# vvvm23/distributed-pytorch-cookbook

Measured on AMD Instinct MI355X. Metric: tokens/sec (node) GPT-2 training per recipe (DDP/FSDP/PP) at 1/2/4/8 MI355X, higher is better.
Workload: dtype bf16; 1 GPU; model=gpt2-small, global_batch=64, seq_len=1024, parallelism=dp1, recipe=main-ddp.py, reduce_dtype=fp32, pp_comm_dtype=fp32, step_graph=True

## Files before the change

distributed_pytorch_cookbook_amd/models/fused.py:

```python
from __future__ import annotations

import os
from dataclasses import dataclass
from typing import Optional

import torch

from ..ops.attention import attention_bwd, attention_fwd
from ..ops.elementwise import bias_act_bwd
from ..ops.dropout import dropout_residual
from ..ops.embedding import embedding_bwd, embedding_fwd
from ..ops.gemm import (ACT_GELU, ACT_MUL, ACT_NONE, ACT_RELU, act_code, linear_dgrad, linear_fwd, linear_wgrad,
                        register_side_stream)
from ..ops.loss import cross_entropy_fused, cross_entropy_rows
from ..ops.norm import layernorm_bwd, layernorm_fwd

LN_EPS = 1e-5
_DH_F32 = os.environ.get("DPC_DH_F32", "0") == "1"


def _dh_dtype(cdt):
    return torch.float32 if _DH_F32 else cdt


_HEAD_DGRAD_F32 = os.environ.get("DPC_HEAD_DGRAD_F32", "auto")


def _head_dgrad_dtype(T, D, cdt):
    if _HEAD_DGRAD_F32 in ("0", "1"):
        return torch.float32 if _HEAD_DGRAD_F32 == "1" else _dh_dtype(cdt)
    tiles = ((T + 255) // 256) * ((D + 255) // 256)
    return torch.float32 if tiles < 128 else _dh_dtype(cdt)


_HEAD_CHUNK = int(os.environ.get("DPC_HEAD_CHUNK", "0"))


def vocab_ld(vocab: int) -> int:
    return (vocab + 63) // 64 * 64


@dataclass
class LMOutput:
    loss: torch.Tensor
    n_valid: torch.Tensor
    n_correct: Optional[torch.Tensor] = None


def _qkv_weight(store, attn):
    wq, wk, wv = (store.weight(m.weight) for m in (attn.to_q, attn.to_k, attn.to_v))
    n = wq.shape[0]
    if (wk.data_ptr() == wq.data_ptr() + wq.numel() * wq.element_size()
            and wv.data_ptr() == wk.data_ptr() + wk.numel() * wk.element_size()):
        return wq.as_strided((3 * n, wq.shape[1]), (wq.shape[1], 1))
    return torch.cat([wq, wk, wv], 0)


def _head_weight_padded(store, head, rows: int):
    w = store.weight(head.weight)
    V, D = w.shape
    if rows == V or getattr(head.weight, "_dpc_pad_rows", 0) == 0 or w.stride() != (D, 1):
        return w
    end = w.storage_offset() + rows * D
    if end * w.element_size() > w.untyped_storage().nbytes():
        return w
    return w.as_strided((rows, D), (D, 1))
# ... 141 lines not shown

_FUSE_TAIL = os.environ.get("DPC_FUSE_FFN_TAIL", "1") == "1"
_FUSE_FFN_LN = os.environ.get("DPC_FUSE_FFN_LN", "1") == "1"


def _tail_ok(x, cdt):
    return _FUSE_TAIL and (cdt == torch.bfloat16 or not x.is_cuda)


class _LayerFn(torch.autograd.Function):

    @staticmethod
    def forward(ctx, x, mask, layer, store, N, S, act, training, drops=(None, None), recompute=False,
                prev_tail=None, tail=None):
        u = layer._unit_id
        store.pre_forward(u)
        pre = None
        if prev_tail is not None and prev_tail.pending is not None:
            pre, prev_tail.pending = prev_tail.pending, None
        fuse = tail if (tail is not None and tail.fuse_next) else None
        x3, saved = _layer_forward(x, mask, layer, store, N, S, act, training and not recompute, drops,
                                   pre=pre, fuse_out=fuse)
        store.post_forward(u, training)
        if training:
            ctx.save_for_backward(x, mask, *(saved or ()))
            ctx.layer, ctx.store, ctx.dims, ctx.act = layer, store, (N, S), act
            ctx.drops, ctx.recompute = drops, recompute
            ctx.fused_out = fuse is not None
            ctx.prev_tail, ctx.tail = prev_tail, tail
            if tail is not None and saved is not None and _tail_ok(x, store.compute_dtype):
                tail.z2, tail.act, tail.drop = saved[-1], act, drops[1]
                bias = layer.fc.down_proj.bias
                tail.bias_grad = lambda: store.grad(bias)
        return x3

    @staticmethod
    def backward(ctx, dx3):
        x, mask, *saved = ctx.saved_tensors
        layer, store, act = ctx.layer, ctx.store, ctx.act
        N, S = ctx.dims
        H, hd = layer.attn.heads, layer.attn.head_dim
        store.pre_backward(layer._unit_id)
        if ctx.recompute:
            _, saved = _layer_forward(x, mask, layer, store, N, S, act, True, ctx.drops,
                                      fuse_out=_FfnTail() if ctx.fused_out else None)
        dx = _layer_backward(dx3, x, mask, saved, layer, store, N, S, H, hd, act, ctx.drops,
                             ctx.prev_tail, ctx.tail)
        u = layer._unit_id
        _w(lambda: store.post_backward(u))
        return dx, None, None, None, None, None, None, None, None, None, None, None


_WGRAD_STREAM = os.environ.get("DPC_WGRAD_STREAM", "0") == "1"
_side_streams: dict = {}


class _SideWork:
    def __init__(self, device: torch.device):
        self.on = _WGRAD_STREAM and device.type == "cuda"
        self.stream = None
        if self.on:
            key = torch.cuda.current_stream(device).cuda_stream
            if key not in _side_streams:
                _side_streams[key] = torch.cuda.Stream(device=device)
                register_side_stream(_side_streams[key])
            self.stream = _side_streams[key]

    def run(self, fn, *tensors):
        if _W_DEFER is not None:
            _W_DEFER.append(fn)
            return
        if not self.on:
            fn()
            return
        self.stream.wait_stream(torch.cuda.current_stream(self.stream.device))
        with torch.cuda.stream(self.stream):
            fn()
        for t in tensors:
            t.record_stream(self.stream)

    def join(self):
        if self.on:
            torch.cuda.current_stream(self.stream.device).wait_stream(self.stream)


def _layer_backward(dx3, x, mask, saved, layer, store, N, S, H, hd, act, drops, prev_tail=None, tail=None):
    (h1, mu1, rs1, qkv, o, lse, x2, h2, mu2, rs2, zup, uact, z2) = saved
    attn, fc = layer.attn, layer.fc
    w, g = store.weight, store.grad
    cdt = store.compute_dtype
    drop_attn, drop_ffn = drops
    dx = dx3.contiguous()
    side = _SideWork(dx.device)
    if tail is not None and tail.dz2 is not None:
        dz2 = tail.dz2
        tail.dz2 = None
    else:
        dz2 = bias_act_bwd(dx, z2, act, g(fc.down_proj.bias), out_dtype=cdt, drop=drop_ffn)
    side.run(lambda: linear_wgrad(dz2, uact, out=g(fc.down_proj.weight)), dz2, uact)
    dz1 = linear_dgrad(dz2, w(fc.down_proj.weight), act_bwd=ACT_MUL if act == ACT_GELU else act, aux_in=zup,
                       out_dtype=cdt, colsum=g(fc.up_proj.bias))
    side.run(lambda: linear_wgrad(dz1, h2, out=g(fc.up_proj.weight)), dz1, h2)
    dh2 = linear_dgrad(dz1, w(fc.up_proj.weight), out_dtype=_dh_dtype(cdt))
    dyo = torch.empty(dx.shape, device=dx.device, dtype=cdt)
    layernorm_bwd(dh2, x2, mu2, rs2, w(layer.norm2.weight), dx, g(layer.norm2.weight),
                  g(layer.norm2.bias), gout=dyo, gsum=g(attn.to_out.bias), drop=drop_attn)
    side.run(lambda: linear_wgrad(dyo, o, out=g(attn.to_out.weight)), dyo, o)
    do = linear_dgrad(dyo, w(attn.to_out.weight), out_dtype=cdt)
    dqkv = attention_bwd(do, qkv, o, lse, N, S, H, hd, mask, causal=True)
    gqkv, split = _qkv_grad(store, attn)

    def qkv_wgrad():
        linear_wgrad(dqkv, h1, out=gqkv)
        if split is not None:
            n = split[0].shape[0]
            for i, gi in enumerate(split):
                gi.add_(gqkv[i * n:(i + 1) * n])

    side.run(qkv_wgrad, dqkv, h1, gqkv)
    dh1 = linear_dgrad(dqkv, _qkv_weight(store, attn), out_dtype=_dh_dtype(cdt))
    kw = {}
    if prev_tail is not None:
        prev_tail.consume(kw, x.shape[0], x.shape[1], x.device, cdt)
    layernorm_bwd(dh1, x, mu1, rs1, w(layer.norm1.weight), dx, g(layer.norm1.weight),
                  g(layer.norm1.bias), **kw)
    side.join()
    return dx


def _ln_in(x, pending, gamma, beta, cdt):
    if pending is None:
        return layernorm_fwd(x, gamma, beta, LN_EPS, cdt)
    x2p, z2p, dropp, actp = pending
    return layernorm_fwd(x2p, gamma, beta, LN_EPS, cdt, add=(z2p, None, dropp, actp), x_out=x)


_unit_ln = {}


def materialize_pending(x, tail) -> None:
    if tail is None or tail.pending is None:
        return
    pending, tail.pending = tail.pending, None
    D = x.shape[1]
    key = (x.device, D)
    if key not in _unit_ln:
        _unit_ln[key] = (torch.ones(D, device=x.device), torch.zeros(D, device=x.device))
    g, b = _unit_ln[key]
    with torch.no_grad():
        _ln_in(x, pending, g, b, pending[1].dtype)


class _HeadFn(torch.autograd.Function):

    @staticmethod
    def forward(ctx, x, targets, norm, head, store, unit, training, want_correct, prev_tail=None):
        store.pre_forward(unit)
        w = store.weight
        cdt = store.compute_dtype
        V = w(head.weight).shape[0]
        T = x.shape[0]
        pending = None
        if prev_tail is not None and prev_tail.pending is not None:
            pending, prev_tail.pending = prev_tail.pending, None
        hf, mu, rs = _ln_in(x, pending, w(norm.weight), w(norm.bias), cdt)
        ld = vocab_ld(V) if x.is_cuda else V
        buf = torch.empty(T, ld, device=x.device, dtype=cdt)
        wpad = _head_weight_padded(store, head, ld)
        chunk = _HEAD_CHUNK if (x.is_cuda and cdt == torch.bfloat16) else 0
        if chunk and T > chunk:
            tg = targets.reshape(-1)
            n_valid = (tg != -100).sum().float()
            inv = 1.0 / n_valid.clamp_min(1.0)
            row_loss = torch.empty(T, device=x.device, dtype=torch.float32)
            row_corr = torch.empty(T, device=x.device, dtype=torch.float32) if want_correct else None
            for c0 in range(0, T, chunk):
                c1 = min(T, c0 + chunk)
                linear_fwd(hf[c0:c1], wpad, out=buf[c0:c1])
# ... 124 lines not shown
```

distributed_pytorch_cookbook_amd/ops/_lib.py:

```python
from __future__ import annotations

import ctypes
import os
import threading
from ctypes import c_float, c_int, c_longlong, c_uint, c_void_p

import torch

from . import build as _build

P = c_void_p
LL = c_longlong


class GemmArgs(ctypes.Structure):
    _fields_ = [
        ("A", P), ("B", P), ("C", P), ("bias", P), ("residual", P), ("aux_in", P),
        ("aux_out", P), ("alpha_ptr", P), ("colsum", P),
        ("lda", LL), ("ldb", LL), ("ldc", LL), ("ldr", LL), ("ld_aux_in", LL), ("ld_aux_out", LL),
        ("M", c_int), ("N", c_int), ("K", c_int),
        ("alpha", c_float),
        ("act", c_int), ("act_bwd", c_int), ("out_f32", c_int), ("accumulate", c_int),
        ("a_kmaj", c_int), ("b_kmaj", c_int),
        ("a_r", c_int), ("a_c", c_int), ("b_r", c_int), ("b_c", c_int),
# ... 187 lines not shown
    "dpc_decode_attn": DecodeAttnArgs,
    "dpc_gemv": GemvArgs,
    "dpc_sample": SampleArgs,
    "dpc_embedding_bwd_sorted": EmbBwdArgs,
    "dpc_gemm": GemmArgs,
    "dpc_gemm_f32": GemmArgs,
    "dpc_attn_fwd": AttnArgs,
    "dpc_attn_bwd": AttnArgs,
    "dpc_attn_fwd_f32": AttnArgs,
    "dpc_attn_bwd_f32": AttnArgs,
    "dpc_layernorm_fwd": LNArgs,
    "dpc_layernorm_bwd": LNArgs,
    "dpc_embedding_fwd": EmbArgs,
    "dpc_embedding_bwd": EmbArgs,
    "dpc_cross_entropy": CEArgs,
    "dpc_adamw": AdamArgs,
    "dpc_amp_check": AmpCheckArgs,
    "dpc_amp_update": AmpUpdateArgs,
    "dpc_grad_sumsq": GradSumsqArgs,
    "dpc_clip_coef": ClipCoefArgs,
    "dpc_cast_f32_bf16": CastArgs,
    "dpc_bias_act_bwd": BiasActArgs,
    "dpc_dropout_residual": DropResArgs,
}

_lock = threading.Lock()
_lib = None
_error = None


def lib() -> ctypes.CDLL:
    global _lib, _error
    if _lib is not None:
        return _lib
    if _error is not None:
        raise RuntimeError(f"kernel library unavailable: {_error}")
    with _lock:
        if _lib is None:
            if _build.needs_build():
                try:
                    _build.build()
                except Exception as exc:
                    _error = exc
                    raise
            handle = ctypes.CDLL(str(_build.LIB_PATH), mode=ctypes.RTLD_GLOBAL)
            for name, st in _FUNCS.items():
                fn = getattr(handle, name)
                fn.argtypes = [ctypes.POINTER(st), c_void_p]
                fn.restype = c_int
            handle.dpc_gemm_set_impl.argtypes = [c_int]
            handle.dpc_gemm_set_impl.restype = None
            handle.dpc_gemm_explain.argtypes = [ctypes.POINTER(GemmArgs), ctypes.c_char_p, c_int]
            handle.dpc_gemm_explain.restype = c_int
            handle.dpc_gemm_last_kernel.argtypes = []
            handle.dpc_gemm_last_kernel.restype = c_int
            handle.dpc_gemm_set_xcd_split.argtypes = [c_int]
            handle.dpc_gemm_set_xcd_split.restype = None
            handle.dpc_gemm_set_splits.argtypes = [c_int]
            handle.dpc_gemm_set_splits.restype = None
            handle.dpc_set_cu_reserve.argtypes = [c_int]
            handle.dpc_set_cu_reserve.restype = None
            handle.dpc_get_cu_reserve.argtypes = []
            handle.dpc_get_cu_reserve.restype = c_int
            handle.dpc_occupy.argtypes = [c_int, ctypes.c_longlong, c_void_p, c_void_p]
            handle.dpc_occupy.restype = c_int
            handle.dpc_embedding_bwd_ws.argtypes = [c_int, c_int]
            handle.dpc_embedding_bwd_ws.restype = ctypes.c_ulonglong
            handle.dpc_grad_sumsq_max_blocks.argtypes = []
            handle.dpc_grad_sumsq_max_blocks.restype = c_int
            handle.dpc_grad_sumsq_trip.argtypes = []
            handle.dpc_grad_sumsq_trip.restype = ctypes.c_longlong
            if (handle.dpc_grad_sumsq_max_blocks(), handle.dpc_grad_sumsq_trip()) != (SUMSQ_MAX_BLOCKS, SUMSQ_TRIP):
                raise RuntimeError("kernel library: dpc_grad_sumsq geometry differs from ops/_lib.py")
            handle.dpc_ipc_alloc.argtypes = [ctypes.c_longlong, c_int, ctypes.POINTER(c_void_p)]
            handle.dpc_ipc_free.argtypes = [c_void_p]
            handle.dpc_ipc_handle.argtypes = [c_void_p, c_void_p]
            handle.dpc_ipc_open.argtypes = [c_void_p, ctypes.POINTER(c_void_p)]
            handle.dpc_ipc_close.argtypes = [c_void_p]
            handle.dpc_ipc_coll.argtypes = [ctypes.POINTER(IpcCollArgs), c_void_p]
            handle.dpc_ipc_p2p.argtypes = [ctypes.POINTER(IpcP2PArgs), c_void_p]
            for f in ("dpc_ipc_alloc", "dpc_ipc_free", "dpc_ipc_handle", "dpc_ipc_open", "dpc_ipc_close",
                      "dpc_ipc_coll", "dpc_ipc_p2p", "dpc_ipc_handle_size", "dpc_ipc_max_world", "dpc_ipc_groups"):
                getattr(handle, f).restype = c_int
            _lib = handle
    return _lib


forced_gemm_impl = -1


def set_gemm_impl(impl: int) -> None:
    global forced_gemm_impl
    forced_gemm_impl = int(impl)
    lib().dpc_gemm_set_impl(int(impl))


def gemm_last_kernel() -> int:
    return int(lib().dpc_gemm_last_kernel())


def gemm_explain(args: GemmArgs) -> str:
    buf = ctypes.create_string_buffer(1024)
    lib().dpc_gemm_explain(ctypes.byref(args), buf, len(buf))
    return buf.value.decode()


def set_gemm_splits(n: int) -> None:
    lib().dpc_gemm_set_splits(int(n))


def set_gemm_xcd_split(on: bool) -> None:
    lib().dpc_gemm_set_xcd_split(int(bool(on)))


def set_cu_reserve(r: int) -> None:
    lib().dpc_set_cu_reserve(int(r))


def get_cu_reserve() -> int:
    return int(lib().dpc_get_cu_reserve())


def occupy(nwg: int, ns: int, sink: torch.Tensor, stream=None) -> None:
    s = (stream or torch.cuda.current_stream()).cuda_stream
    rc = lib().dpc_occupy(int(nwg), int(ns), sink.data_ptr(), s)
    if rc != 0:
        raise RuntimeError(f"dpc_occupy failed: hipError {rc}")


def is_loaded() -> bool:
    return _lib is not None


def stream_ptr(device: torch.device | None = None) -> int:
    return torch.cuda.current_stream(device).cuda_stream


SERIALIZE = os.environ.get("DPC_SERIALIZE", "0") == "1"


def enable_serialize() -> None:
    global SERIALIZE
    SERIALIZE = True
    os.environ["DPC_SERIALIZE"] = "1"
    for k, v in (("AMD_SERIALIZE_KERNEL", "3"), ("AMD_SERIALIZE_COPY", "3"), ("HIP_LAUNCH_BLOCKING", "1")):
        os.environ.setdefault(k, v)


def call(name: str, args: ctypes.Structure, device: torch.device | None = None) -> None:
    rc = getattr(lib(), name)(ctypes.byref(args), stream_ptr(device))
    if rc != 0:
        raise RuntimeError(f"{name} launch failed: hipError {rc}")
    if SERIALIZE and not torch.cuda.is_current_stream_capturing():
        try:
            torch.cuda.current_stream(device).synchronize()
        except RuntimeError as exc:
            raise RuntimeError(f"{name} failed on the device: {exc}") from exc


# ... 3 lines not shown
```

distributed_pytorch_cookbook_amd/ops/build.py:

```python
from __future__ import annotations

import argparse
import os
import shutil
import subprocess
import sys
from concurrent.futures import ThreadPoolExecutor
from pathlib import Path

HERE = Path(__file__).resolve().parent
CSRC = HERE / "csrc"
BUILD_DIR = HERE / "_build"
LIB_PATH = HERE / "libdpc_kernels.so"
ARCH = os.environ.get("DPC_OFFLOAD_ARCH", "gfx950")

SOURCES = ["gemm.hip", "gemm_f32.hip", "attention.hip", "attention_f32.hip", "layernorm.hip", "misc.hip",
           "decode.hip", "sample.hip", "embed_bwd.hip", "ipc_coll.hip"] + sorted(p.name for p in CSRC.glob("gemm7_part*.hip"))
HEADERS = ["common.h", "gemm.h", "gemm_plan.h", "gemm7_kern.h", "gemm9_kern.h", "gemm7_extern.inc"]

CFLAGS = [
    f"--offload-arch={ARCH}",
    "-O3",
    "-std=c++17",
    "-fPIC",
    "-mcode-object-version=5",
    "-ffp-contract=fast",
    "-Wno-unused-result",
]


def hipcc() -> str:
    for cand in (os.environ.get("HIPCC"), shutil.which("hipcc"), "/opt/rocm/bin/hipcc"):
        if cand and Path(cand).exists():
            return cand
    raise RuntimeError("hipcc not found: cannot build the gfx950 kernel library")


FILE_FLAGS = {"attention.hip": ["-fno-honor-nans", "-fno-slp-vectorize"], "attention_f32.hip": ["-fno-honor-nans"]}


HASH_PATH = LIB_PATH.with_suffix(".so.srchash")


def source_hash() -> str:
    import hashlib

    h = hashlib.sha256((" ".join(CFLAGS) + repr(sorted(FILE_FLAGS.items()))).encode())
    for name in SOURCES + HEADERS:
        h.update(name.encode())
        h.update((CSRC / name).read_bytes())
    return h.hexdigest()


def needs_build() -> bool:
    if not LIB_PATH.exists() or not HASH_PATH.exists():
        return True
    return HASH_PATH.read_text().strip() != source_hash()


def _compile(src: Path, obj: Path, verbose: bool) -> None:
    cmd = [hipcc(), *CFLAGS, *FILE_FLAGS.get(src.name, []), "-c", str(src), "-o", str(obj)]
    if verbose:
        print(" ".join(cmd), flush=True)
    r = subprocess.run(cmd, capture_output=True, text=True)
    if r.returncode != 0:
        raise RuntimeError(f"hipcc failed for {src.name}:\n{r.stdout}\n{r.stderr}")


def _deps(name: str, seen=None) -> set:
    import re
# ... 68 lines not shown
```

distributed_pytorch_cookbook_amd/ops/csrc/gemm.hip:

```cpp
#include "gemm9_kern.h"
#define G7_SIG (dpc::GemmArgs, unsigned long long, unsigned long long, dpc::G7Plan)
#define G7_INST(F, K, ...) extern template __global__ void dpc::K<__VA_ARGS__> G7_SIG;
#include "gemm7_extern.inc"
#undef G7_INST

#include <cstdio>
#include <cstdlib>
#include <cstring>

namespace dpc {


struct TileSlot {
  int bid, split, splits;
};
__device__ __forceinline__ TileSlot tile_slot(const GemmArgs& p, int ntiles) {
  TileSlot t;
  if (p.ksplit < -1) {
    t.splits = -p.ksplit;
    t.split = blockIdx.x % t.splits;
    t.bid = blockIdx.x / t.splits;
    return t;
  }
  t.splits = p.ksplit > 1 ? p.ksplit : 1;
// ... 623 lines not shown
  }
}

#define DPC_BY_LAYOUT(ak, bk, K, ...)                                                            \
  ((ak) ? ((bk) ? K<__VA_ARGS__ true, true> : K<__VA_ARGS__ true, false>)                        \
        : ((bk) ? K<__VA_ARGS__ false, true> : K<__VA_ARGS__ false, false>))

static int gemm_run(const GemmPlan& p, const GemmArgs& a, hipStream_t stream) {
  g_last_kernel = p.last_kernel;
  if (p.rc != 0) return p.rc;
  GemmArgs b = a;
  b.ksplit = p.ksplit;
  b.nt_store = p.nt_store;
  if (p.drop_ws) b.ws = nullptr;
  const GemmKernelId& k = p.kernel;
  const dim3 grid(p.grid), block(p.block);
  for (int i = 0; i < p.nsteps; ++i) {
    switch (p.steps[i]) {
      case GS_CLEAR:
        (void)hipMemset2DAsync(a.C, (size_t)a.ldc * 4, 0, (size_t)a.N * 4, (size_t)a.M, stream);
        break;
      case GS_SPLITK_REDUCE:
        hipLaunchKernelGGL(g7_splitk_reduce, dim3(p.red_x), dim3(256), 0, stream, static_cast<float*>(a.C), a.ldc,
                           static_cast<const float*>(a.ws), a.M, a.N, p.g7.splits, a.accumulate, p.nt_store & 2);
        break;
      case GS_COLSUM_REDUCE:
        hipLaunchKernelGGL(g7_colsum_reduce, dim3(p.red_x, p.red_y), dim3(256), 0, stream, a.colsum,
                           static_cast<const float*>(a.ws), 2 * p.g7.tiles_m, a.N);
        break;
      case GS_KERNEL:
        if (k.family >= GK_V7) {
          const G7KernelFn fn = g7_kernel_fn(k);
          if (!fn) return (int)hipErrorInvalidDeviceFunction;
          hipLaunchKernelGGL(fn, grid, block, 0, stream, b, p.a_bytes, p.b_bytes, p.g7);
        } else if (k.family == GK_V1) {
          hipLaunchKernelGGL(DPC_BY_LAYOUT(k.t[0], k.t[1], gemm_kernel, ), grid, block, 0, stream, b);
        } else {
          void (*fn)(GemmArgs, unsigned long long, unsigned long long) = nullptr;
          if (k.family == GK_V2 && k.t[0] == 64 && k.t[1] == 2) fn = DPC_BY_LAYOUT(k.t[2], k.t[3], gemm2_kernel, 64, 2, );
          else if (k.family == GK_V2 && k.t[0] == 64 && k.t[1] == 3) fn = DPC_BY_LAYOUT(k.t[2], k.t[3], gemm2_kernel, 64, 3, );
          else if (k.family == GK_V2 && k.t[0] == 32 && k.t[1] == 3) fn = DPC_BY_LAYOUT(k.t[2], k.t[3], gemm2_kernel, 32, 3, );
          else if (k.family == GK_V3 && k.t[0] == 256 && k.t[1] == 128 && k.t[4] == 32 && k.t[5] == 3)
            fn = DPC_BY_LAYOUT(k.t[6], k.t[7], gemm3_kernel, 256, 128, 4, 2, 32, 3, );
          if (!fn) return (int)hipErrorInvalidDeviceFunction;
          hipLaunchKernelGGL(fn, grid, block, 0, stream, b, p.a_bytes, p.b_bytes);
        }
        break;
      default: break;
    }
  }
  return (int)hipGetLastError();
}

DPC_API int dpc_gemm(const GemmArgs* a, hipStream_t stream) {
  return gemm_run(gemm_plan(*a, settings_for_launch()), *a, stream);
}

DPC_API int dpc_gemm_explain(const GemmArgs* a, char* buf, int cap) {
  return gemm_plan_text(gemm_plan(*a, settings_for_launch()), buf, cap);
}
```

distributed_pytorch_cookbook_amd/ops/csrc/gemm_plan.h:

```cpp
#pragma once
#include <algorithm>
#include <cstdint>
#include <cstdio>

namespace dpc {

struct GemmArgs {
  const void* A;
  const void* B;
  void* C;
  const float* bias;
  const float* residual;
  const void* aux_in;
  void* aux_out;
  const float* alpha_ptr;
  float* colsum;
  long long lda, ldb, ldc, ldr, ld_aux_in, ld_aux_out;
  int M, N, K;
  float alpha;
  int act;
  int act_bwd;
  int out_f32;
  int accumulate;
  int a_kmaj, b_kmaj;
  int a_r, a_c, b_r, b_c;
  int ksplit;
  int impl;
  int aux_f32;
  void* ws;
  long long ws_bytes;
  int nt_store;
  int aux_deriv;
};

struct G7Plan {
  int tiles_m, tiles_n;
  int tile_n;
  int units;
  int grid;
  int nk;
  int nk_all;
  int splits;
  int store_cnt;
  int debug;
};

constexpr int GP_ACT_GELU = 2, GP_ACT_MUL = 3, GP_G7_KB = 32;

struct GemmSettings {
  int impl = -1;
  int force_splits = 0;
  int xcd_split = 0;
  int policy[5] = {0, 0, 0, 0, 0};
  int nt_store = 77;
  int act_lds = -1, act_lds_env = 1;
  int res_lds = -1, res_lds_env = 1;
  int cus = 256, cu_reserve = 0;
};

enum GemmFamily { GF_V1, GF_V2, GF_V3, GF_V7, GF_V8, GF_V7D, GF_V9 };
struct GemmImpl {
  int id;
  const char* name;
  int family;
  int kb, stages;
  int tile_m, tile_n;
  int wgs;
  int dma;
  bool persistent;
};
constexpr GemmImpl GEMM_IMPLS[] = {
    {1, "v1", GF_V1, 64, 1, 128, 128, 2, 0, false},
    {2, "v2-64x2", GF_V2, 64, 2, 128, 128, 2, 0, false},
    {3, "v2-64x3", GF_V2, 64, 3, 128, 128, 1, 0, false},
    {4, "v2-32x3", GF_V2, 32, 3, 128, 128, 3, 0, false},
    {10, "v3-256x128", GF_V3, 32, 3, 256, 128, 1, 0, false},
    {16, "v7-dma0", GF_V7, 32, 5, 256, 256, 1, 0, true},
    {17, "v7-unit", GF_V7, 32, 5, 256, 256, 1, 2, false},
    {19, "v7-dma1", GF_V7, 32, 5, 256, 256, 1, 1, true},
    {20, "v7", GF_V7, 32, 5, 256, 256, 1, 2, true},
    {21, "v8", GF_V8, 32, 5, 256, 128, 2, 2, true},
    {22, "v7-pair", GF_V7, 32, 5, 256, 256, 1, 3, true},
    {23, "v7-quad", GF_V7, 32, 5, 256, 256, 1, 4, true},
    {24, "v7d", GF_V7D, 32, 5, 256, 256, 1, 5, true},
    {25, "v7-split", GF_V7, 32, 5, 256, 256, 1, 6, true},
    {26, "v9", GF_V9, 64, 2, 256, 256, 1, 7, true},
};
inline const GemmImpl* gemm_impl_row(int id) {
  for (const GemmImpl& r : GEMM_IMPLS)
    if (r.id == id) return &r;
  return nullptr;
}

enum GemmKernelFamily { GK_NONE, GK_V1, GK_V2, GK_V3, GK_V7, GK_V7D, GK_V9 };
struct GemmKernelId {
  int family;
  int t[8];
// ... 259 lines not shown
    p.kernel = {GK_V2, {row.kb, row.stages, ak, bk, 0, 0, 0, 0}};
    p.block = 256;
  } else {
    p.kernel = {GK_V3, {row.tile_m, row.tile_n, 4, 2, row.kb, row.stages, ak, bk}};
    p.block = 512;
  }
  add_step(p, GS_KERNEL);
}

}

inline GemmPlan gemm_plan(const GemmArgs& a, const GemmSettings& st) {
  using namespace plan_detail;
  GemmPlan p;
  if (a.M <= 0 || a.N <= 0) return p;
  if (a.aux_deriv && (!a.aux_out || a.act != GP_ACT_GELU)) { p.rc = -1; return p; }
  p.a_bytes = (unsigned long long)operand_bytes(a.a_r, a.a_c, a.lda);
  p.b_bytes = (unsigned long long)operand_bytes(a.b_r, a.b_c, a.ldb);
  p.nt_store = st.nt_store;
  const bool v2_ok = gemm2_ok(a);
  const bool plain = plain_epilogue(a);
  const int pol = policy_impl(a, st);
  int impl = st.impl;
  if (impl < 0 && a.impl > 0) impl = a.impl;
  if (impl < 0 && pol <= 0 && gemm7_ok(a)) {
    if (plain) impl = 20;
    else if (a.a_kmaj && a.b_kmaj && !a.residual && !a.accumulate && !a.aux_in && !a.colsum && !a.act_bwd &&
             a.K % 64 == 0 && a.K >= 192)
      impl = 26;
  }
  if (impl < 0) {
    impl = 1;
    if (v2_ok) {
      impl = 2;
      if (a.a_kmaj && a.b_kmaj && a.K <= 1024) impl = 10;
      else if (a.a_kmaj && !a.b_kmaj && a.K <= 1024) impl = 10;
      else if (a.a_kmaj && !a.b_kmaj && a.K <= 2304) impl = 4;
      else if (!a.a_kmaj && !a.b_kmaj && a.M > 2304 && a.M <= 4096) impl = 4;
      if (pol > 0) impl = pol;
    }
  }
  if (st.impl < 0 && a.impl <= 0 && v2_ok && plain && a.out_f32 && !a.a_kmaj && !a.b_kmaj && pol <= 0 && impl != 20)
    impl = 2;
  if (impl < 2) impl = 1;
  const GemmImpl* row = gemm_impl_row(impl);
  if (row && row->family >= GF_V7) {
    if (plan7(a, st, *row, p)) return p;
    row = gemm_impl_row(2);
  }
  if (!row) { p.rc = 1; return p; }
  if (!v2_ok) row = gemm_impl_row(1);
  plan123(a, st, *row, p);
  return p;
}

inline int gemm_plan_text(const GemmPlan& p, char* buf, int cap) {
  int n = 0;
  auto put = [&](const char* fmt, auto... v) {
    if (n < cap) n += snprintf(buf + n, (size_t)(cap - n), fmt, v...);
  };
  auto puts = [&](const char* s) { put("%s", s); };
  auto tf = [](int v) { return v ? "true" : "false"; };
  if (p.rc) put("rc=%d", p.rc);
  for (int i = 0; i < p.nsteps; ++i) {
    if (i) puts("; ");
    const GemmKernelId& k = p.kernel;
    const G7Plan& g = p.g7;
    switch (p.steps[i]) {
      case GS_CLEAR: puts("clear"); break;
      case GS_SPLITK_REDUCE: put("splitk_reduce grid=%u", p.red_x); break;
      case GS_COLSUM_REDUCE: put("colsum_reduce grid=%ux%u", p.red_x, p.red_y); break;
      case GS_KERNEL:
        if (k.family == GK_V1) put("gemm_kernel<%s, %s>", tf(k.t[0]), tf(k.t[1]));
        else if (k.family == GK_V2) put("gemm2_kernel<%d, %d, %s, %s>", k.t[0], k.t[1], tf(k.t[2]), tf(k.t[3]));
        else if (k.family == GK_V3)
          put("gemm3_kernel<%d, %d, %d, %d, %d, %d, %s, %s>", k.t[0], k.t[1], k.t[2], k.t[3], k.t[4], k.t[5], tf(k.t[6]), tf(k.t[7]));
        else if (k.family == GK_V7) put("gemm7_kernel<%d, %d, %s, %s, %d, %d>", k.t[0], k.t[1], tf(k.t[2]), tf(k.t[3]), k.t[4], k.t[5]);
        else if (k.family == GK_V7D) put("gemm7d_kernel<%d, %d, %s, %s>", k.t[0], k.t[1], tf(k.t[2]), tf(k.t[3]));
        else put("gemm9_kernel<%d, %s, %s, %d, %d>", k.t[0], tf(k.t[1]), tf(k.t[2]), k.t[3], k.t[4]);
        if (k.family >= GK_V7)
          put(" g7=%d,%d,%d,%d,%d,%d,%d,%d,%d,%d", g.tiles_m, g.tiles_n, g.tile_n, g.units, g.grid, g.nk, g.nk_all, g.splits,
              g.store_cnt, g.debug);
        else put(" grid=%u", p.grid);
        if (p.block != 256) put(" block=%u", p.block);
        if (p.ksplit) put(" ksplit=%d", p.ksplit);
        if (p.nt_store != 77) put(" nt=%d", p.nt_store);
        if (p.drop_ws) puts(" wsdrop");
        break;
      default: break;
    }
  }
  put(" | last=%d", p.last_kernel);
  return n < cap ? n : cap - 1;
}

}
```

distributed_pytorch_cookbook_amd/ops/gemm.py:

```python
from __future__ import annotations

import atexit
import json
import math
import os

import torch
import torch.nn.functional as F

from . import _lib

ACT_NONE, ACT_RELU, ACT_GELU = 0, 1, 2
ACT_MUL = 3
ACTS = {None: ACT_NONE, "none": ACT_NONE, "relu": ACT_RELU, "gelu": ACT_GELU}


def act_code(act) -> int:
    if isinstance(act, int):
        return act
    return ACTS[act]


def act_fwd_ref(v: torch.Tensor, act: int) -> torch.Tensor:
    if act == ACT_RELU:
# ... 322 lines not shown
    if (x.is_cuda and x.shape[0] <= _GEMV_ROWS and aux_out is None and x.dtype == torch.bfloat16
            and w.dtype == torch.bfloat16):
        return _linear_fwd_few_rows(x, w, bias, act_code(act), residual, out, out_dtype)
    return gemm(x, w, a_kmaj=True, b_kmaj=True, bias=bias, act=act, residual=residual,
                aux_out=aux_out, out=out, out_dtype=out_dtype, aux_deriv=aux_deriv)


_GEMV_ROWS = 16
_GEMV_NATIVE = os.environ.get("DPC_GEMV", "1") == "1"


def _gemv_ok(x, w, bias, residual, out, N):
    return (x.stride(1) == 1 and w.stride(1) == 1 and x.shape[1] % 8 == 0 and x.stride(0) % 8 == 0
            and w.stride(0) % 8 == 0 and x.data_ptr() % 16 == 0 and w.data_ptr() % 16 == 0
            and (bias is None or (bias.dtype == torch.float32 and bias.is_contiguous()))
            and (residual is None or (residual.dtype == torch.float32 and residual.stride(1) == 1))
            and out.stride(1) == 1 and w.shape[0] <= N)


def _linear_fwd_few_rows(x, w, bias, act, residual, out, out_dtype):
    M, K = x.shape
    Nw = w.shape[0]
    if out is None:
        out = torch.empty(M, Nw, device=x.device, dtype=out_dtype)
    N = out.shape[1]
    if _GEMV_NATIVE and _gemv_ok(x, w, bias, residual, out, N) and out.dtype in (torch.float32, torch.bfloat16):
        args = _lib.GemvArgs(
            x=x.data_ptr(), w=w.data_ptr(), bias=_lib.ptr(bias), residual=_lib.ptr(residual),
            y=out.data_ptr(), ldx=x.stride(0), ldw=w.stride(0),
            ldr=residual.stride(0) if residual is not None else 0, ldy=out.stride(0),
            M=M, N=N, Nw=Nw, K=K, act=act, y_f32=int(out.dtype == torch.float32))
        _lib.call("dpc_gemv", args, x.device)
        return out
    v = torch.mm(x, w.t()) if bias is None else torch.addmm(bias.to(x.dtype), x, w.t())
    if act:
        v = act_fwd_ref(v, act)
    if residual is not None:
        v = residual + v.to(residual.dtype)
    out[:, :Nw].copy_(v)
    if N > Nw:
        out[:, Nw:].zero_()
    return out


def linear_dgrad(dy, w, *, act_bwd=None, aux_in=None, out=None, out_dtype=torch.bfloat16,
                 alpha_t=None, colsum=None):
    return gemm(dy, w, a_kmaj=True, b_kmaj=False, act_bwd=act_bwd, aux_in=aux_in, out=out,
                out_dtype=out_dtype, alpha_t=alpha_t, colsum=colsum)


def linear_wgrad(dy, x, *, out, accumulate=True, alpha_t=None):
    return gemm(dy, x, a_kmaj=False, b_kmaj=False, out=out, accumulate=accumulate,
                alpha_t=alpha_t)
```

Measured before the change: 1.026 million tokens/s.

## Group per-layer weight-gradient GEMMs into one persistent split-K launch

Collects the four weight-gradient GEMMs of each transformer layer backward (down, up, out-proj, qkv) and runs them through a new grouped gemm7 kernel. All tiles share one persistent grid with split-K, and a single grouped reduction kernel adds the partials into the fp32 grads. The aim is to cut per-GEMM launch overhead and the tail underutilization of small wgrad GEMMs on 256 CUs. In exchange the wgrads are deferred to the end of the layer backward, so they lose interleaving with the dgrads. If the plan rejects the shapes it falls back to the individual GEMMs.

```diff
diff --git a/distributed_pytorch_cookbook_amd/models/fused.py b/distributed_pytorch_cookbook_amd/models/fused.py
--- a/distributed_pytorch_cookbook_amd/models/fused.py
+++ b/distributed_pytorch_cookbook_amd/models/fused.py
@@ -11,7 +11,7 @@
 from ..ops.dropout import dropout_residual
 from ..ops.embedding import embedding_bwd, embedding_fwd
 from ..ops.gemm import (ACT_GELU, ACT_MUL, ACT_NONE, ACT_RELU, act_code, linear_dgrad, linear_fwd, linear_wgrad,
-                        register_side_stream)
+                        linear_wgrad_group, register_side_stream)
 from ..ops.loss import cross_entropy_fused, cross_entropy_rows
 from ..ops.norm import layernorm_bwd, layernorm_fwd
 
@@ -259,6 +259,7 @@
 
 
 _WGRAD_STREAM = os.environ.get("DPC_WGRAD_STREAM", "0") == "1"
+_WGRAD_GROUP = os.environ.get("DPC_WGRAD_GROUP", "1") == "1"
 _side_streams: dict = {}
 
 
@@ -299,20 +300,28 @@
     drop_attn, drop_ffn = drops
     dx = dx3.contiguous()
     side = _SideWork(dx.device)
+    group = [] if _WGRAD_GROUP else None
+
+    def wgrad(dy_, x_, out_):
+        if group is not None:
+            group.append((dy_, x_, out_, True, None))
+        else:
+            side.run(lambda: linear_wgrad(dy_, x_, out=out_), dy_, x_)
+
     if tail is not None and tail.dz2 is not None:
         dz2 = tail.dz2
         tail.dz2 = None
     else:
         dz2 = bias_act_bwd(dx, z2, act, g(fc.down_proj.bias), out_dtype=cdt, drop=drop_ffn)
-    side.run(lambda: linear_wgrad(dz2, uact, out=g(fc.down_proj.weight)), dz2, uact)
+    wgrad(dz2, uact, g(fc.down_proj.weight))
     dz1 = linear_dgrad(dz2, w(fc.down_proj.weight), act_bwd=ACT_MUL if act == ACT_GELU else act, aux_in=zup,
                        out_dtype=cdt, colsum=g(fc.up_proj.bias))
-    side.run(lambda: linear_wgrad(dz1, h2, out=g(fc.up_proj.weight)), dz1, h2)
+    wgrad(dz1, h2, g(fc.up_proj.weight))
     dh2 = linear_dgrad(dz1, w(fc.up_proj.weight), out_dtype=_dh_dtype(cdt))
     dyo = torch.empty(dx.shape, device=dx.device, dtype=cdt)
     layernorm_bwd(dh2, x2, mu2, rs2, w(layer.norm2.weight), dx, g(layer.norm2.weight),
                   g(layer.norm2.bias), gout=dyo, gsum=g(attn.to_out.bias), drop=drop_attn)
-    side.run(lambda: linear_wgrad(dyo, o, out=g(attn.to_out.weight)), dyo, o)
+    wgrad(dyo, o, g(attn.to_out.weight))
     do = linear_dgrad(dyo, w(attn.to_out.weight), out_dtype=cdt)
     dqkv = attention_bwd(do, qkv, o, lse, N, S, H, hd, mask, causal=True)
     gqkv, split = _qkv_grad(store, attn)
@@ -324,13 +333,18 @@
             for i, gi in enumerate(split):
                 gi.add_(gqkv[i * n:(i + 1) * n])
 
-    side.run(qkv_wgrad, dqkv, h1, gqkv)
+    if group is not None and split is None:
+        group.append((dqkv, h1, gqkv, True, None))
+    else:
+        side.run(qkv_wgrad, dqkv, h1, gqkv)
     dh1 = linear_dgrad(dqkv, _qkv_weight(store, attn), out_dtype=_dh_dtype(cdt))
     kw = {}
     if prev_tail is not None:
         prev_tail.consume(kw, x.shape[0], x.shape[1], x.device, cdt)
     layernorm_bwd(dh1, x, mu1, rs1, w(layer.norm1.weight), dx, g(layer.norm1.weight),
                   g(layer.norm1.bias), **kw)
+    if group:
+        side.run(lambda: linear_wgrad_group(group), *(t for it in group for t in it[:2]))
     side.join()
     return dx
 
diff --git a/distributed_pytorch_cookbook_amd/ops/_lib.py b/distributed_pytorch_cookbook_amd/ops/_lib.py
--- a/distributed_pytorch_cookbook_amd/ops/_lib.py
+++ b/distributed_pytorch_cookbook_amd/ops/_lib.py
@@ -263,6 +263,10 @@
             handle.dpc_gemm_set_impl.restype = None
             handle.dpc_gemm_explain.argtypes = [ctypes.POINTER(GemmArgs), ctypes.c_char_p, c_int]
             handle.dpc_gemm_explain.restype = c_int
+            handle.dpc_gemm_group.argtypes = [ctypes.POINTER(GemmArgs), c_int, c_void_p]
+            handle.dpc_gemm_group.restype = c_int
+            handle.dpc_gemm_group_explain.argtypes = [ctypes.POINTER(GemmArgs), c_int, ctypes.c_char_p, c_int]
+            handle.dpc_gemm_group_explain.restype = c_int
             handle.dpc_gemm_last_kernel.argtypes = []
             handle.dpc_gemm_last_kernel.restype = c_int
             handle.dpc_gemm_set_xcd_split.argtypes = [c_int]
@@ -316,6 +320,31 @@
     return buf.value.decode()
 
 
+GEMM_GROUP_MAX = 8
+
+
+def gemm_group(items: list, device: torch.device | None = None) -> bool:
+    arr = (GemmArgs * len(items))(*items)
+    rc = lib().dpc_gemm_group(arr, len(items), stream_ptr(device))
+    if rc == -1:
+        return False
+    if rc != 0:
+        raise RuntimeError(f"dpc_gemm_group launch failed: hipError {rc}")
+    if SERIALIZE and not torch.cuda.is_current_stream_capturing():
+        try:
+            torch.cuda.current_stream(device).synchronize()
+        except RuntimeError as exc:
+            raise RuntimeError(f"dpc_gemm_group failed on the device: {exc}") from exc
+    return True
+
+
+def gemm_group_explain(items: list) -> str:
+    arr = (GemmArgs * len(items))(*items)
+    buf = ctypes.create_string_buffer(1024)
+    lib().dpc_gemm_group_explain(arr, len(items), buf, len(buf))
+    return buf.value.decode()
+
+
 def set_gemm_splits(n: int) -> None:
     lib().dpc_gemm_set_splits(int(n))
 
diff --git a/distributed_pytorch_cookbook_amd/ops/build.py b/distributed_pytorch_cookbook_amd/ops/build.py
--- a/distributed_pytorch_cookbook_amd/ops/build.py
+++ b/distributed_pytorch_cookbook_amd/ops/build.py
@@ -15,7 +15,8 @@
 ARCH = os.environ.get("DPC_OFFLOAD_ARCH", "gfx950")
 
 SOURCES = ["gemm.hip", "gemm_f32.hip", "attention.hip", "attention_f32.hip", "layernorm.hip", "misc.hip",
-           "decode.hip", "sample.hip", "embed_bwd.hip", "ipc_coll.hip"] + sorted(p.name for p in CSRC.glob("gemm7_part*.hip"))
+           "decode.hip", "sample.hip", "embed_bwd.hip", "ipc_coll.hip", "gemm7_group.hip"] + sorted(
+               p.name for p in CSRC.glob("gemm7_part*.hip"))
 HEADERS = ["common.h", "gemm.h", "gemm_plan.h", "gemm7_kern.h", "gemm9_kern.h", "gemm7_extern.inc"]
 
 CFLAGS = [
diff --git a/distributed_pytorch_cookbook_amd/ops/csrc/gemm.hip b/distributed_pytorch_cookbook_amd/ops/csrc/gemm.hip
--- a/distributed_pytorch_cookbook_amd/ops/csrc/gemm.hip
+++ b/distributed_pytorch_cookbook_amd/ops/csrc/gemm.hip
@@ -699,6 +699,11 @@
   return (int)hipGetLastError();
 }
 
+namespace dpc {
+const GemmSettings& gemm_settings_for_launch() { return settings_for_launch(); }
+void gemm_note_last_kernel(int code) { g_last_kernel = code; }
+}
+
 DPC_API int dpc_gemm(const GemmArgs* a, hipStream_t stream) {
   return gemm_run(gemm_plan(*a, settings_for_launch()), *a, stream);
 }
diff --git a/distributed_pytorch_cookbook_amd/ops/csrc/gemm7_group.hip b/distributed_pytorch_cookbook_amd/ops/csrc/gemm7_group.hip
--- /dev/null
+++ b/distributed_pytorch_cookbook_amd/ops/csrc/gemm7_group.hip
@@ -0,0 +1,329 @@
+#include "gemm7_kern.h"
+
+namespace dpc {
+
+struct G7Item {
+  const void* A;
+  const void* B;
+  const float* alpha_ptr;
+  unsigned long long a_bytes, b_bytes;
+  long long lda, ldb;
+  long long slab_off;
+  int M, N, tiles_m, tiles_n;
+  int tile0;
+  float alpha;
+};
+struct G7Group {
+  long long slab_elems;
+  int n;
+  G7Item item[G7_GROUP_MAX];
+};
+
+__global__ __launch_bounds__(256, 1) void gemm7_group_kernel(GemmArgs p, G7Plan pl, G7Group grp) {
+  constexpr int NJ = 8, NL = G7_NL, NP = 2 * NL, SLOT = G7_SLOT, NS = 5, DIST = NS - 1;
+  static_assert(NS * SLOT * 2 <= 160 * 1024, "LDS");
+  __shared__ __attribute__((aligned(16))) bf16_t smem[NS * SLOT];
+
+  const int lane = threadIdx.x & 63;
+  const int wid = __builtin_amdgcn_readfirstlane(threadIdx.x >> 6);
+  const int wr = wid >> 1, wc = wid & 1;
+  const int ar = wr * 128, bc = wc * 128;
+
+  const int local = g7_local(blockIdx.x, pl.grid);
+  const int nmine = local < pl.units ? (pl.units - local + pl.grid - 1) / pl.grid : 0;
+  if (nmine == 0) return;
+
+  auto lane_now = []() {
+    int l;
+    asm volatile("v_mbcnt_lo_u32_b32 %0, -1, 0\n\tv_mbcnt_hi_u32_b32 %0, -1, %0" : "=v"(l));
+    return l;
+  };
+  auto find_item = [&](int tile) {
+    int it = 0;
+    for (int i = 1; i < grp.n; ++i) it = tile >= grp.item[i].tile0 ? i : it;
+    return it;
+  };
+  auto item_tile = [&](const G7Item& g, int tile, int& m0, int& n0) {
+    G7Plan ip = pl;
+    ip.tiles_m = g.tiles_m;
+    ip.tiles_n = g.tiles_n;
+    g7_tile(ip, tile - g.tile0, m0, n0);
+  };
+
+  int va[NL], vb[NL];
+  dma_offsets3<32, false, NL>(va, 0, wid, lane);
+  dma_offsets3<32, false, NL>(vb, 0, wid, lane);
+  unsigned long long a_step = 0, b_step = 0, a_bytes = 0, b_bytes = 0;
+  const void* is_A = nullptr;
+  const void* is_B = nullptr;
+  long long is_lda = 0, is_ldb = 0;
+  int is_u = 0, is_k = 0, is_slot = 0;
+  unsigned long long is_aoff = 0, is_boff = 0;
+  int is_kt0 = 0;
+  const int ntiles = pl.tiles_m * pl.tiles_n;
+  auto set_org = [&](int ui) {
+    const int uu = local + ui * pl.grid;
+    const int sp = uu / ntiles;
+    const int t = uu - sp * ntiles;
+    const G7Item& g = grp.item[find_item(t)];
+    is_A = g.A;
+    is_B = g.B;
+    a_bytes = g.a_bytes;
+    b_bytes = g.b_bytes;
+    if (g.lda != is_lda) {
+      const int d = (int)(g.lda - is_lda) * 2, kr0 = 16 * (wid & 1) + (lane_now() >> 4);
+#pragma unroll
+      for (int i = 0; i < NL; ++i) va[i] += d * (kr0 + 4 * i);
+      is_lda = g.lda;
+      a_step = 32ull * is_lda * 2;
+    }
+    if (g.ldb != is_ldb) {
+      const int d = (int)(g.ldb - is_ldb) * 2, kr0 = 16 * (wid & 1) + (lane_now() >> 4);
+#pragma unroll
+      for (int i = 0; i < NL; ++i) vb[i] += d * (kr0 + 4 * i);
+      is_ldb = g.ldb;
+      b_step = 32ull * is_ldb * 2;
+    }
+    int m0, n0;
+    item_tile(g, t, m0, n0);
+    is_kt0 = sp * pl.nk;
+    is_aoff = (unsigned long long)m0 * 2 + a_step * is_kt0;
+    is_boff = (unsigned long long)n0 * 2 + b_step * is_kt0;
+  };
+  set_org(0);
+  __amdgpu_buffer_rsrc_t rsa, rsb;
+  const bf16_t* is_lds = smem;
+  auto prep = [&]() {
+    const bool valid = is_u < nmine && is_kt0 + is_k < pl.nk_all;
+    const unsigned long long la = a_bytes - is_aoff, lb = b_bytes - is_boff;
+    const unsigned na = valid ? ((la >> 32) ? 0xffffffffu : (unsigned)la) : 0u;
+    const unsigned nb = valid ? ((lb >> 32) ? 0xffffffffu : (unsigned)lb) : 0u;
+    rsa = __builtin_amdgcn_make_buffer_rsrc((void*)((const char*)is_A + is_aoff), 0, na, 0x00020000);
+    rsb = __builtin_amdgcn_make_buffer_rsrc((void*)((const char*)is_B + is_boff), 0, nb, 0x00020000);
+    is_lds = smem + is_slot * SLOT;
+  };
+  auto piece2 = [&](int i) {
+    if (i < NL) g7_piece2(rsa, va[i], va[i + 1] - 1024, is_lds + (wid * NL + i) * 512);
+    else g7_piece2(rsb, vb[i - NL], vb[i + 1 - NL] - 1024, is_lds + G7_TA + (wid * NL + i - NL) * 512);
+  };
+  auto advance = [&]() {
+    is_slot = is_slot + 1 == NS ? 0 : is_slot + 1;
+    is_aoff += a_step;
+    is_boff += b_step;
+    if (++is_k == pl.nk) {
+      is_k = 0;
+      ++is_u;
+      if (is_u < nmine) set_org(is_u);
+    }
+  };
+
+#pragma unroll
+  for (int s = 0; s < DIST; ++s) {
+    prep();
+#pragma unroll
+    for (int i = 0; i < NP; i += 2) piece2(i);
+    advance();
+  }
+  prep();
+
+  floatx4 acc[8][NJ];
+
+  g7_wait<(DIST - 1) * NP>();
+  __builtin_amdgcn_s_barrier();
+  asm volatile("" ::: "memory");
+  bf16x8 a0[8], b0[NJ], a1[8], b1[NJ];
+#pragma unroll
+  for (int i = 0; i < 8; ++i) a0[i] = frag3<32, false>(smem, ar + 16 * i, 0, lane);
+#pragma unroll
+  for (int j = 0; j < NJ; ++j) b0[j] = frag3<32, false>(smem + G7_TA, bc + 16 * j, 0, lane);
+  g7_wait<(DIST - 2) * NP>();
+  __builtin_amdgcn_s_barrier();
+  asm volatile("" ::: "memory");
+
+  int rd_slot = 1;
+  int credit = 0;
+
+  auto mf = [&](int i, int j, const bf16x8* ac, const bf16x8* bcur, bool first) G7_AI {
+    acc[i][j] = __builtin_amdgcn_mfma_f32_16x16x32_bf16(bcur[j], ac[i], first ? floatx4{0.f, 0.f, 0.f, 0.f} : acc[i][j],
+                                                        0, 0, 0);
+  };
+  auto dma5 = [&](int i, int step) G7_AI {
+    if (step == 0) {
+      if (i < NL) g7_m0(is_lds + (wid * NL + i) * 512);
+      else g7_m0(is_lds + G7_TA + (wid * NL + i - NL) * 512);
+    } else if (step == 1) {
+      if (i < NL) g7_ld<0>(rsa, va[i]);
+      else g7_ld<0>(rsb, vb[i - NL]);
+    } else {
+      if (i < NL) g7_ld<1024>(rsa, va[i + 1] - 1024);
+      else g7_ld<1024>(rsb, vb[i + 1 - NL] - 1024);
+    }
+  };
+#define G7_SB __builtin_amdgcn_sched_barrier(0)
+#define G7_GROUP5(i, ac, bcur, an, bn, FIRST)                                                        \
+  do {                                                                                              \
+    mf(i, 0, ac, bcur, FIRST); G7_SB;                                                               \
+    an[i] = frag3<32, false>(la_, ar + 16 * i, 0, lane);                                            \
+    G7_SB; mf(i, 1, ac, bcur, FIRST); G7_SB;                                                        \
+    bn[i] = frag3<32, false>(la_ + G7_TA, bc + 16 * i, 0, lane);                                    \
+    G7_SB; mf(i, 2, ac, bcur, FIRST); G7_SB;                                                        \
+    if (!((i) & 1) && (i) < NP) dma5(i, 0);                                                         \
+    if ((i) == 7) advance();                                                                        \
+    G7_SB; mf(i, 3, ac, bcur, FIRST); G7_SB;                                                        \
+    if (!((i) & 1) && (i) < NP) dma5(i, 1);                                                         \
+    G7_SB; mf(i, 4, ac, bcur, FIRST); G7_SB;                                                        \
+    if (!((i) & 1) && (i) < NP) dma5(i, 2);                                                         \
+    G7_SB; mf(i, 5, ac, bcur, FIRST); G7_SB;                                                        \
+    if ((i) == 7) prep();                                                                           \
+    G7_SB; mf(i, 6, ac, bcur, FIRST); G7_SB;                                                        \
+    mf(i, 7, ac, bcur, FIRST); G7_SB;                                                               \
+  } while (0)
+#define G7_BODYC(ac, bcur, an, bn, FIRST, CREDIT)                                                   \
+  do {                                                                                              \
+    const bf16_t* la_ = smem + rd_slot * SLOT;                                                      \
+    G7_GROUP5(0, ac, bcur, an, bn, FIRST); G7_GROUP5(1, ac, bcur, an, bn, FIRST);                   \
+    G7_GROUP5(2, ac, bcur, an, bn, FIRST); G7_GROUP5(3, ac, bcur, an, bn, FIRST);                   \
+    G7_GROUP5(4, ac, bcur, an, bn, FIRST); G7_GROUP5(5, ac, bcur, an, bn, FIRST);                   \
+    G7_GROUP5(6, ac, bcur, an, bn, FIRST); G7_GROUP5(7, ac, bcur, an, bn, FIRST);                   \
+    rd_slot = rd_slot + 1 == NS ? 0 : rd_slot + 1;                                                  \
+    if ((CREDIT) && credit > 0) {                                                                   \
+      --credit;                                                                                     \
+      g7_wait<(DIST - 2) * NP + 47>();                                                              \
+    } else {                                                                                        \
+      g7_wait<(DIST - 2) * NP>();                                                                   \
+    }                                                                                               \
+    __builtin_amdgcn_s_barrier();                                                                   \
+    asm volatile("" ::: "memory");                                                                  \
+  } while (0)
+
+  for (int u = 0; u < nmine; ++u) {
+    G7_BODYC(a0, b0, a1, b1, true, true);
+    G7_BODYC(a1, b1, a0, b0, false, true);
+    for (int k = 2; k < pl.nk; k += 2) {
+      G7_BODYC(a0, b0, a1, b1, false, false);
+      G7_BODYC(a1, b1, a0, b0, false, false);
+    }
+    const int uu = local + u * pl.grid;
+    const int sp = uu / ntiles, t = uu - sp * ntiles;
+    const G7Item& g = grp.item[find_item(t)];
+    int m0, n0;
+    item_tile(g, t, m0, n0);
+    GemmArgs q = p;
+    q.C = static_cast<float*>(p.ws) + (long long)sp * grp.slab_elems + g.slab_off;
+    q.M = g.M;
+    q.N = g.N;
+    q.ldc = g.N;
+    q.out_f32 = 1;
+    q.alpha = g.alpha;
+    q.alpha_ptr = g.alpha_ptr;
+    g7_epilogue<0, NJ>(q, acc, m0 + ar, n0 + bc, lane_now());
+    credit = (pl.store_cnt >= 48 && m0 + 256 <= g.M && n0 + 256 <= g.N) ? DIST - 2 : 0;
+  }
+#undef G7_BODYC
+#undef G7_GROUP5
+#undef G7_SB
+  g7_wait<0>();
+}
+
+struct G7RedItem {
+  float* C;
+  long long ldc;
+  long long slab_off;
+  long long q0;
+  int M, N, accumulate;
+};
+struct G7RedGroup {
+  int n;
+  G7RedItem item[G7_GROUP_MAX];
+};
+
+static __global__ __launch_bounds__(256) void g7_group_reduce(G7RedGroup rg, const float* ws, long long slab, int s,
+                                                               int nt) {
+  const long long stride = (long long)gridDim.x * 256;
+  const long long tid = (long long)blockIdx.x * 256 + threadIdx.x;
+  for (int it = 0; it < rg.n; ++it) {
+    const G7RedItem& g = rg.item[it];
+    const int n4 = g.N >> 2;
+    const long long nq = (long long)g.M * n4;
+    for (long long i = ((tid - g.q0) % stride + stride) % stride; i < nq; i += stride) {
+      const long long m = i / n4, n = (i - m * n4) << 2;
+      const float* w = ws + g.slab_off + m * g.N + n;
+      float4 v = *reinterpret_cast<const float4*>(w);
+      int k = 1;
+      for (; k + 3 < s; k += 4) {
+        const float4 u0 = *reinterpret_cast<const float4*>(w + k * slab);
+        const float4 u1 = *reinterpret_cast<const float4*>(w + (k + 1) * slab);
+        const float4 u2 = *reinterpret_cast<const float4*>(w + (k + 2) * slab);
+        const float4 u3 = *reinterpret_cast<const float4*>(w + (k + 3) * slab);
+        v.x += u0.x; v.y += u0.y; v.z += u0.z; v.w += u0.w;
+        v.x += u1.x; v.y += u1.y; v.z += u1.z; v.w += u1.w;
+        v.x += u2.x; v.y += u2.y; v.z += u2.z; v.w += u2.w;
+        v.x += u3.x; v.y += u3.y; v.z += u3.z; v.w += u3.w;
+      }
+      for (; k < s; ++k) {
+        const float4 u = *reinterpret_cast<const float4*>(w + k * slab);
+        v.x += u.x; v.y += u.y; v.z += u.z; v.w += u.w;
+      }
+      float4* c = reinterpret_cast<float4*>(g.C + m * g.ldc + n);
+      if (g.accumulate) {
+        const float4 o = *c;
+        v.x += o.x; v.y += o.y; v.z += o.z; v.w += o.w;
+      }
+      st16(c, v, nt);
+    }
+  }
+}
+
+const GemmSettings& gemm_settings_for_launch();
+void gemm_note_last_kernel(int code);
+
+}
+
+using namespace dpc;
+
+DPC_API int dpc_gemm_group(const GemmArgs* items, int n, hipStream_t stream) {
+  const G7GroupPlan gp = gemm_group_plan(items, n, gemm_settings_for_launch());
+  if (gp.rc != 0) return -1;
+  G7Group grp = {};
+  G7RedGroup rg = {};
+  grp.n = rg.n = n;
+  grp.slab_elems = gp.slab_elems;
+  for (int i = 0; i < n; ++i) {
+    const GemmArgs& a = items[i];
+    const G7GroupItemPlan& ip = gp.item[i];
+    G7Item& k = grp.item[i];
+    k.A = a.A;
+    k.B = a.B;
+    k.alpha_ptr = a.alpha_ptr;
+    k.a_bytes = (unsigned long long)plan_detail::operand_bytes(a.a_r, a.a_c, a.lda);
+    k.b_bytes = (unsigned long long)plan_detail::operand_bytes(a.b_r, a.b_c, a.ldb);
+    k.lda = a.lda;
+    k.ldb = a.ldb;
+    k.slab_off = ip.slab_off;
+    k.M = a.M;
+    k.N = a.N;
+    k.tiles_m = ip.tiles_m;
+    k.tiles_n = ip.tiles_n;
+    k.tile0 = ip.tile0;
+    k.alpha = a.alpha;
+    G7RedItem& r = rg.item[i];
+    r.C = static_cast<float*>(a.C);
+    r.ldc = a.ldc;
+    r.slab_off = ip.slab_off;
+    r.q0 = ip.slab_off / 4;
+    r.M = a.M;
+    r.N = a.N;
+    r.accumulate = a.accumulate;
+  }
+  GemmArgs shared = items[0];
+  shared.nt_store = gp.nt_store;
+  gemm_note_last_kernel(704);
+  hipLaunchKernelGGL(gemm7_group_kernel, dim3((unsigned)gp.g7.grid), dim3(256), 0, stream, shared, gp.g7, grp);
+  hipLaunchKernelGGL(g7_group_reduce, dim3(gp.red_x), dim3(256), 0, stream, rg, static_cast<const float*>(shared.ws),
+                     gp.slab_elems, gp.g7.splits, gp.nt_store & 2);
+  return (int)hipGetLastError();
+}
+
+DPC_API int dpc_gemm_group_explain(const GemmArgs* items, int n, char* buf, int cap) {
+  return gemm_group_plan_text(gemm_group_plan(items, n, gemm_settings_for_launch()), buf, cap);
+}
diff --git a/distributed_pytorch_cookbook_amd/ops/csrc/gemm_plan.h b/distributed_pytorch_cookbook_amd/ops/csrc/gemm_plan.h
--- a/distributed_pytorch_cookbook_amd/ops/csrc/gemm_plan.h
+++ b/distributed_pytorch_cookbook_amd/ops/csrc/gemm_plan.h
@@ -43,6 +43,22 @@
   int splits;
   int store_cnt;
   int debug;
+};
+
+constexpr int G7_GROUP_MAX = 8;
+struct G7GroupItemPlan {
+  int tiles_m, tiles_n;
+  int tile0;
+  long long slab_off;
+};
+struct G7GroupPlan {
+  int rc = -1;
+  int n = 0;
+  G7Plan g7 = {};
+  G7GroupItemPlan item[G7_GROUP_MAX] = {};
+  long long slab_elems = 0;
+  unsigned red_x = 0;
+  int nt_store = 0;
 };
 
 constexpr int GP_ACT_GELU = 2, GP_ACT_MUL = 3, GP_G7_KB = 32;
@@ -408,6 +424,88 @@
   if (!v2_ok) row = gemm_impl_row(1);
   plan123(a, st, *row, p);
   return p;
+}
+
+inline G7GroupPlan gemm_group_plan(const GemmArgs* items, int n, const GemmSettings& st) {
+  using namespace plan_detail;
+  G7GroupPlan gp;
+  if (n < 1 || n > G7_GROUP_MAX) return gp;
+  const GemmArgs& a0 = items[0];
+  if (!a0.ws || !al(a0.ws, 16) || a0.K <= 0) return gp;
+  GemmSettings split2 = st;
+  split2.force_splits = 2;
+  constexpr GemmKernelId want = {GK_V7, {4, 6, 0, 0, 128, 0, 0, 0}};
+  int tiles = 0;
+  long long elems = 0;
+  for (int i = 0; i < n; ++i) {
+    const GemmArgs& a = items[i];
+    if (a.M <= 0 || a.N <= 0 || a.K != a0.K || a.ws != a0.ws || a.ws_bytes != a0.ws_bytes) return gp;
+    if (a.a_kmaj || a.b_kmaj || !a.out_f32 || !plain_epilogue(a) || !gemm7_ok(a) || !bias_ok(a)) return gp;
+    const GemmPlan one = gemm_plan(a, split2);
+    if (one.rc != 0 || gemm_kernel_key(one.kernel) != gemm_kernel_key(want) || one.nsteps != 2) return gp;
+    G7GroupItemPlan& it = gp.item[i];
+    it.tiles_m = (a.M + 255) / 256;
+    it.tiles_n = (a.N + 255) / 256;
+    it.tile0 = tiles;
+    it.slab_off = elems;
+    tiles += it.tiles_m * it.tiles_n;
+    elems += (long long)a.M * a.N;
+  }
+  const int nk_all = (a0.K + GP_G7_KB - 1) / GP_G7_KB;
+  const int cus = std::max(8, st.cus - st.cu_reserve);
+  auto fits = [&](int c) { return (long long)c * elems * 4 <= a0.ws_bytes; };
+  int s = st.force_splits > 0 ? st.force_splits : 1;
+  if (st.force_splits <= 0) {
+    double best = 1e30;
+    for (int c = 1; c <= 32; ++c) {
+      const int per = 2 * ((nk_all + 2 * c - 1) / (2 * c));
+      if (c > 1 && per < 16) break;
+      const int rounds = (tiles * c + cus - 1) / cus;
+      double cost = (double)rounds * per;
+      if (c > 1) {
+        if (!fits(c)) continue;
+        double red_us = 0.0;
+        for (int i = 0; i < n; ++i) red_us += (double)(c + 1 + items[i].accumulate) * items[i].M * items[i].N * 4 / 5e6;
+        cost += rounds * 12.0 + red_us / 0.7;
+      }
+      if (cost < best - 1e-9) { best = cost; s = c; }
+    }
+  }
+  if (s < 2 || !fits(s)) return gp;
+  G7Plan& pl = gp.g7;
+  pl.tiles_m = tiles;
+  pl.tiles_n = 1;
+  pl.tile_n = 256;
+  pl.nk_all = nk_all;
+  pl.splits = s;
+  pl.nk = 2 * ((nk_all + 2 * s - 1) / (2 * s));
+  pl.units = tiles * s;
+  pl.grid = pl.units > cus ? cus : pl.units;
+  pl.store_cnt = 64;
+  pl.debug = 0;
+  gp.n = n;
+  gp.slab_elems = elems;
+  gp.red_x = (unsigned)std::min<long long>((elems / 4 + 255) / 256, 4096);
+  gp.nt_store = st.nt_store;
+  gp.rc = 0;
+  return gp;
+}
+
+inline int gemm_group_plan_text(const G7GroupPlan& p, char* buf, int cap) {
+  int n = 0;
+  auto put = [&](const char* fmt, auto... v) {
+    if (n < cap) n += snprintf(buf + n, (size_t)(cap - n), fmt, v...);
+  };
+  if (p.rc) {
+    put("rc=%d", p.rc);
+  } else {
+    const G7Plan& g = p.g7;
+    put("group g7=%d,%d,%d,%d,%d,%d,%d,%d,%d,%d slab=%lld red=%u |", g.tiles_m, g.tiles_n, g.tile_n, g.units, g.grid, g.nk,
+        g.nk_all, g.splits, g.store_cnt, g.debug, p.slab_elems, p.red_x);
+    for (int i = 0; i < p.n; ++i)
+      put(" %d:%dx%d@%lld", p.item[i].tile0, p.item[i].tiles_m, p.item[i].tiles_n, p.item[i].slab_off);
+  }
+  return n < cap ? n : cap - 1;
 }
 
 inline int gemm_plan_text(const GemmPlan& p, char* buf, int cap) {
diff --git a/distributed_pytorch_cookbook_amd/ops/gemm.py b/distributed_pytorch_cookbook_amd/ops/gemm.py
--- a/distributed_pytorch_cookbook_amd/ops/gemm.py
+++ b/distributed_pytorch_cookbook_amd/ops/gemm.py
@@ -398,3 +398,45 @@
 def linear_wgrad(dy, x, *, out, accumulate=True, alpha_t=None):
     return gemm(dy, x, a_kmaj=False, b_kmaj=False, out=out, accumulate=accumulate,
                 alpha_t=alpha_t)
+
+
+def _wgrad_args(dy, x, out, accumulate, alpha_t, ws):
+    if not (dy.is_cuda and dy.dtype == torch.bfloat16 and x.dtype == torch.bfloat16
+            and out.dtype == torch.float32 and dy.dim() == 2 and x.dim() == 2 and out.dim() == 2):
+        return None
+    K = max(dy.shape[0], x.shape[0])
+    M, N = out.shape
+    if dy.shape[1] > M or x.shape[1] > N:
+        raise ValueError(f"wgrad group: incompatible operands dy{tuple(dy.shape)} x{tuple(x.shape)} -> ({M},{N})")
+    if out.stride(1) != 1:
+        raise ValueError(f"wgrad group: bad out {tuple(out.shape)} stride {out.stride()}")
+    _check_operand(dy, dy.shape[0], dy.shape[1], "A")
+    _check_operand(x, x.shape[0], x.shape[1], "B")
+    args = _lib.GemmArgs(
+        A=dy.data_ptr(), B=x.data_ptr(), C=out.data_ptr(), alpha_ptr=_lib.ptr(alpha_t),
+        lda=dy.stride(0), ldb=x.stride(0), ldc=out.stride(0), M=M, N=N, K=K, alpha=1.0,
+        out_f32=1, accumulate=int(accumulate), a_kmaj=0, b_kmaj=0,
+        a_r=dy.shape[0], a_c=dy.shape[1], b_r=x.shape[0], b_c=x.shape[1],
+        ws=_lib.ptr(ws), ws_bytes=ws.numel() * 4,
+    )
+    if _table and _lib.forced_gemm_impl < 0:
+        key = _sig(M, N, K, False, False, True, None, ACT_NONE, ACT_NONE, None, None, None, accumulate)
+        impl = _table.get(key)
+        if impl is None and _NEAR:
+            impl = _near(key)
+        args.impl = impl or 0
+    return args
+
+
+def linear_wgrad_group(items) -> None:
+    items = list(items)
+    for c0 in range(0, len(items), _lib.GEMM_GROUP_MAX):
+        chunk = items[c0:c0 + _lib.GEMM_GROUP_MAX]
+        ws = _workspace(chunk[0][0].device) if chunk[0][0].is_cuda else None
+        args = [None]
+        if ws is not None:
+            args = [_wgrad_args(dy, x, out, acc, alpha_t, ws) for dy, x, out, acc, alpha_t in chunk]
+        if all(a is not None for a in args) and _lib.gemm_group(args, chunk[0][0].device):
+            continue
+        for dy, x, out, acc, alpha_t in chunk:
+            linear_wgrad(dy, x, out=out, accumulate=acc, alpha_t=alpha_t)
```

Measured after the change: 1.026 million tokens/s. Within noise of the previous version (-0.0%).
